# facebookresearch/SlowFast

Hardware: AMD Instinct MI355X
Metric: clips/sec (fwd+bwd), SlowFast-8x8-R50 32x224^2 synthetic clips, per-GPU batch 32 (higher is better)
Workload: dtype fp16; 1 GPU; SLOWFAST_8x8_R50: forward + cross_entropy loss + backward + sgd step, inputs resident in HBM, per-GPU batch 32; global_batch=32, parallelism=dp1, launch=hip-graph(fwd+bwd) + eager all-reduce/optimizer, optimizer=FlatOptimizer (fused unscale+norm+clip+update, dynamic loss scale on device)

## Files before the change

### include/sfamd.h

```cpp
#ifndef SFAMD_H
#define SFAMD_H
#include <stddef.h>
#include <stdint.h>
#ifdef __cplusplus
extern "C" {
#endif

#define SF_ABI_VERSION 35
typedef void* sf_stream_t;

typedef struct sf_conv_desc {
    int32_t N, Ci, Ti, Hi, Wi;
    int32_t Co, To, Ho, Wo;
    int32_t kT, kH, kW;
    int32_t sT, sH, sW;
    int32_t pT, pH, pW;
    int32_t dT, dH, dW;
    int32_t Cw;
    int32_t ldx, ldy;
    int32_t Cow;
} sf_conv_desc;

int sf_abi_version(void);
const char* sf_backend(void);
#define SF_ACT_FP16 0
#define SF_ACT_BF16_ID 1
int sf_act_dtype(void);
const char* sf_last_error(void);
const char* sf_build_id(void);

int sf_conv_weight_ld(const sf_conv_desc* d, int32_t* ldf, int32_t* ldd);
// ... 12 lines not shown
int sf_conv_fwd_mtiles(const sf_conv_desc* d);
int sf_conv_fwd(const sf_conv_desc* d, const void* x, const void* wf, const float* in_scale, const float* in_shift,
                int in_relu, const float* bias, void* y, float* stat_part, sf_stream_t stream);
int sf_conv_fwd_fused(const sf_conv_desc* d, const void* x, const void* wf, const float* bias, const void* resid,
                      int32_t ldr, int out_relu, void* y, sf_stream_t stream);
int sf_conv_dgrad(const sf_conv_desc* d, const void* dy, const void* wd, const void* resid, int32_t ldr,
                  const void* resid_bits, void* dx, sf_stream_t stream);
int sf_conv_dgrad_bn(const sf_conv_desc* d, const void* dy, const void* wd, const void* resid, int32_t ldr,
                     const void* resid_bits, void* dx, const float* mask_scale, const float* mask_shift,
                     const void* mask_bits, const void* bn_y, int32_t bn_ldy, float* bn_part, int32_t bn_part_rows,
                     int32_t* bn_rows, sf_stream_t stream);
int64_t sf_conv_wgrad_workspace(const sf_conv_desc* d);
int64_t sf_conv_wgrad_rowtab_bytes(const sf_conv_desc* d);
int sf_conv_wgrad_rowtab(const sf_conv_desc* d, void* tab, sf_stream_t stream);
int sf_conv_wgrad(const sf_conv_desc* d, const void* x, const float* in_scale, const float* in_shift, int in_relu,
                  const void* dy, float* dw, float out_scale, int zero_first, void* workspace, int64_t workspace_bytes,
                  const void* rowtab, sf_stream_t stream);
int sf_conv_c_bwd_plan(const sf_conv_desc* d, int in_affine, int mask_bits, int32_t* tile_rows, int64_t* workspace_bytes);
int sf_conv_c_bwd(const sf_conv_desc* d, const void* dz, int32_t lddz, const void* mask_bits, const void* yc, int32_t ldyc,
                  const float* coef, const void* act, const void* wd, const float* bn_scale, const float* bn_shift,
                  const void* bn_y, int32_t bn_ldy, float* bn_part, int32_t bn_part_rows, int32_t* bn_rows, void* d_in,
                  int32_t ld_in, float* dw, float out_scale, int zero_first, void* workspace, int64_t workspace_bytes,
                  sf_stream_t stream);

int sf_bn_finalize(float* part, int32_t nblk, int32_t C, int32_t Creal, float count, const float* gamma, const float* beta,
                   float* running_mean, float* running_var, float momentum, float eps, float* scale, float* shift,
                   float* save_mean, float* save_rstd, sf_stream_t stream);
int sf_bn_act(int64_t M, int32_t C, const void* y, int32_t ldy, const float* scale, const float* shift, const void* r,
              int32_t ldr, const float* rscale, const float* rshift, int relu, void* out, int32_t ldo, void* mask_out,
              sf_stream_t stream);
int sf_bn_bwd_blocks(int64_t M, int32_t C);
int sf_bn_bwd_reduce(int64_t M, int32_t C, const void* dz, int32_t lddz, const void* zmask, int32_t ldm, const void* y,
                     int32_t ldy, const float* scale, const float* shift, int relu_self, float* part,
                     sf_stream_t stream);
int sf_bn_bwd_finalize(float* part, int32_t nblk, int32_t C, int32_t Creal, float count, const float* gamma, const float* mean,
                       const float* rstd, float inv_loss_scale, float* dgamma, float* dbeta, int accumulate,
                       float* coef, sf_stream_t stream);
int sf_bn_bwd_apply(int64_t M, int32_t C, const void* dz, int32_t lddz, const void* zmask, int32_t ldm, const void* y,
                    int32_t ldy, const float* scale, const float* shift, int relu_self, const float* coef, void* dy,
                    int32_t lddy, void* gout, int32_t ldg, sf_stream_t stream);

int sf_pool_fwd(int32_t N, int32_t T, int32_t H, int32_t W, int32_t C, int32_t kH, int32_t kW, int32_t sH, int32_t sW,
                int32_t pH, int32_t pW, const void* y, int32_t ldy, const float* scale, const float* shift, int relu,
                void* out, int32_t ldo, void* argmax, int32_t cls, sf_stream_t stream);
int sf_pool_bwd(int32_t N, int32_t T, int32_t H, int32_t W, int32_t C, int32_t kH, int32_t kW, int32_t sH, int32_t sW,
                int32_t pH, int32_t pW, const void* pooled, int32_t ldp, const void* argmax, int relu,
// ... 262 lines not shown
```

### slowfast_amd/csrc/sf_api.hip

```cpp
#include "../../include/sfamd.h"
#include "sf_bn.h"
#include "sf_common.h"
#include "sf_igemm.h"
#include "sf_igemm2.h"
#include "sf_wgrad2.h"
#include "sf_cbwd.h"
#include "sf_pool.h"
#include "sf_dwconv.h"
#include "sf_dwsweep.h"
#include "sf_dwtemporal.h"
#include "sf_tokens.h"
#include "sf_x3d.h"
#include "sf_stem.h"
#include "sf_attn.h"
#include "sf_roi.h"
#include "sf_optim.h"
#include "sf_mixup.h"
#include "sf_erase.h"
#include "sf_pack.h"
#include "sf_sample.h"
#include "sf_color.h"
#include "sf_randaug.h"
#include "sf_sslcolor.h"
#include "sf_hog.h"
// ... 865 lines not shown
    int cip, cop, R;
    size_t ws_bytes;
};
#define SF_CBWD_MAX_WGS 1024
template <int CIP, int COP>
static void cbwd_fill(CbwdPlan& w) {
    using K = CbwdCfg<CIP, COP>;
    w.R = K::R;
    w.ws_bytes = (size_t)SF_CBWD_MAX_WGS * COP * CIP * 4;
}
#define SF_CBWD_FOR_SHAPE(cip, cop, ...)                                                         \
    do {                                                                                         \
        if ((cip) == 16 && (cop) == 32) { constexpr int CIP_ = 16, COP_ = 32; __VA_ARGS__; }            \
        else if ((cip) == 16 && (cop) == 64) { constexpr int CIP_ = 16, COP_ = 64; __VA_ARGS__; }       \
        else if ((cip) == 16 && (cop) == 128) { constexpr int CIP_ = 16, COP_ = 128; __VA_ARGS__; }     \
        else if ((cip) == 16 && (cop) == 256) { constexpr int CIP_ = 16, COP_ = 256; __VA_ARGS__; }     \
        else if ((cip) == 32 && (cop) == 32) { constexpr int CIP_ = 32, COP_ = 32; __VA_ARGS__; }       \
        else if ((cip) == 32 && (cop) == 64) { constexpr int CIP_ = 32, COP_ = 64; __VA_ARGS__; }       \
        else if ((cip) == 32 && (cop) == 128) { constexpr int CIP_ = 32, COP_ = 128; __VA_ARGS__; }     \
        else if ((cip) == 32 && (cop) == 256) { constexpr int CIP_ = 32, COP_ = 256; __VA_ARGS__; }     \
        else if ((cip) == 64 && (cop) == 32) { constexpr int CIP_ = 64, COP_ = 32; __VA_ARGS__; }       \
        else if ((cip) == 64 && (cop) == 64) { constexpr int CIP_ = 64, COP_ = 64; __VA_ARGS__; }       \
        else if ((cip) == 64 && (cop) == 128) { constexpr int CIP_ = 64, COP_ = 128; __VA_ARGS__; }     \
        else { constexpr int CIP_ = 64, COP_ = 256; __VA_ARGS__; }                                      \
    } while (0)
static CbwdPlan plan_cbwd(const sf_conv_desc* d, bool in_affine, bool mask_bits) {
    CbwdPlan w;
    memset(&w, 0, sizeof(w));
    if (test_hook("SF_CBWD", 1) == 0) return w;
    if (d->kT != 1 || d->kH != 1 || d->kW != 1 || d->sT != 1 || d->sH != 1 || d->sW != 1 || d->pT || d->pH || d->pW) return w;
    if (d->To != d->Ti || d->Ho != d->Hi || d->Wo != d->Wi) return w;
    if (d->Ci % 8 || d->Ci > 64 || d->Co % 32 || d->Co > 256) return w;
    if (in_affine || !mask_bits) return w;
    w.cip = d->Ci <= 16 ? 16 : d->Ci <= 32 ? 32 : 64;
    w.cop = d->Co <= 32 ? 32 : d->Co <= 64 ? 64 : d->Co <= 128 ? 128 : 256;
    SF_CBWD_FOR_SHAPE(w.cip, w.cop, (cbwd_fill<CIP_, COP_>(w)));
    w.ok = true;
    return w;
}

extern "C" int sf_conv_c_bwd_plan(const sf_conv_desc* d, int in_affine, int mask_bits, int32_t* tile_rows,
                                  int64_t* workspace_bytes) {
    if (check_desc(d)) return -1;
    const CbwdPlan w = plan_cbwd(d, in_affine != 0, mask_bits != 0);
    if (tile_rows) *tile_rows = w.ok ? 128 : 0;
    if (workspace_bytes) *workspace_bytes = w.ok ? (int64_t)w.ws_bytes : 0;
    return w.ok ? 1 : 0;
}
// ... 10 lines not shown
    REQUIRE(lddz >= d->Co && lddz % 8 == 0 && ldyc >= d->Co && ldyc % 8 == 0 && ld_in >= d->Ci && ld_in % 8 == 0,
            "sf_conv_c_bwd: bad row pitch");
    REQUIRE((((uintptr_t)dz | (uintptr_t)yc | (uintptr_t)act | (uintptr_t)wd | (uintptr_t)d_in | (uintptr_t)workspace) & 15) == 0,
            "sf_conv_c_bwd: operands must be 16-byte aligned");
    REQUIRE(workspace_bytes >= (int64_t)w.ws_bytes, "sf_conv_c_bwd: workspace too small (%lld < %lld bytes)",
            (long long)workspace_bytes, (long long)w.ws_bytes);
    const int64_t M = (int64_t)d->N * d->Ti * d->Hi * d->Wi;
    const int ntiles = cdiv(M, 128);
    const bool fuse = bn_part != nullptr;
    if (fuse) {
        REQUIRE(bn_scale && bn_shift && bn_y && bn_rows, "sf_conv_c_bwd: the fused reduction needs bn_scale, bn_shift, bn_y and bn_rows");
        REQUIRE(bn_ldy >= d->Ci && bn_ldy % 8 == 0 && ((uintptr_t)bn_y & 15) == 0, "sf_conv_c_bwd: bad bn_y pitch / alignment");
        REQUIRE(bn_part_rows >= ntiles, "sf_conv_c_bwd: the partial table needs ceil(positions / tile_rows) rows of [2][Ci] floats");
    }
    int32_t ldf, ldd;
    sf_conv_weight_ld(d, &ldf, &ldd);
    CbwdParams p;
    memset(&p, 0, sizeof(p));
    p.M = (int)M; p.Ci = d->Ci; p.Co = d->Co;
    p.dz = (const f16*)dz; p.lddz = lddz; p.bits = (const uint8_t*)mask_bits; p.yc = (const f16*)yc; p.ldyc = ldyc;
    p.coef = coef; p.act = (const f16*)act; p.ldact = d->ldx; p.wd = (const f16*)wd; p.ldw = ldd;
    if (fuse) { p.bnb_y = (const f16*)bn_y; p.bnb_ld = bn_ldy; p.bnb_scale = bn_scale; p.bnb_shift = bn_shift; p.bnb_part = bn_part; }
    p.dx = (f16*)d_in; p.lddx = ld_in; p.ws = (float*)workspace; p.tiles128 = ntiles;
    int wgs;
    const WgradPlan w2 = plan_conv_wgrad(d, false);
    const int forced = test_hook("SF_CBWD_WGS", 0);
    if (forced > 0) {
        wgs = forced < SF_CBWD_MAX_WGS ? forced : SF_CBWD_MAX_WGS;
        p.rps = roundup(cdiv(M, wgs), 32);
        wgs = cdiv(M, p.rps);
    } else if (w2.path == WGRAD_ROWTAB && w2.thin && w2.splits <= SF_CBWD_MAX_WGS) {
        wgs = w2.splits; p.rps = 0;
    } else {
        const WgradPlan w1 = plan_wgrad1(d);
        wgs = w1.splits; p.rps = w1.chunks_per_split * 32;
        REQUIRE(wgs <= SF_CBWD_MAX_WGS, "sf_conv_c_bwd: %d splits", wgs);
    }
    hipStream_t s = (hipStream_t)stream;
    SF_CBWD_FOR_SHAPE(w.cip, w.cop, hipLaunchKernelGGL((sf_cbwd_kernel<CIP_, COP_>), dim3(wgs), dim3(SF_THREADS), 0, s, p));
    if (check_launch("conv_c_bwd")) return -1;
    if (bn_rows) *bn_rows = fuse ? ntiles : 0;
    launch_wgrad_reduce(d, (const float*)workspace, wgs, w.cop, w.cip, false, dw, out_scale, zero_first, s);
    return check_launch("conv_c_bwd_reduce");
}

static RowTile make_rowtile(int64_t M, int C, int max_blocks, dim3& grid) {
    RowTile rt;
    rt.M = (int)M; rt.C = C;
    const int G = C / 8;
    const int TG = G < SF_THREADS ? G : SF_THREADS;
    const int rpi = SF_THREADS / TG;
    int passes = cdiv(M, (int64_t)rpi * max_blocks);
    if (passes < 1) passes = 1;
    rt.rows_per_block = rpi * passes;
    grid = dim3(cdiv(M, rt.rows_per_block), cdiv(G, SF_THREADS));
    return rt;
}
static int check_rows(const char* who, int64_t M, int C) {
    REQUIRE(M > 0 && M < (1ll << 31), "%s: bad row count", who);
    REQUIRE(C > 0 && C % 8 == 0, "%s: C must be a positive multiple of 8 (got %d)", who, C);
    return 0;
}

static const int kFoldAbove = tune_knob("SF_FOLD_ABOVE", 2048);
static int fold_partials(float* part, int& nblk, int C, hipStream_t s) {
    if (nblk <= kFoldAbove || nblk <= 256) return 1;
// ... 2470 lines not shown
```

### slowfast_amd/csrc/sf_cbwd.h

```cpp
#pragma once
#include "sf_bn.h"
#include "sf_common.h"
#include "sf_igemm.h"

struct CbwdParams {
    int M, Ci, Co;
    const f16* dz; int lddz;
    const uint8_t* bits;
    const f16* yc; int ldyc;
    const float* coef;
    const f16* act; int ldact;
    const f16* wd; int ldw;
    const f16* bnb_y; int bnb_ld;
    const float* bnb_scale; const float* bnb_shift;
    float* bnb_part;
    f16* dx; int lddx;
    float* ws;
    int rps;
    int tiles128;
};

template <int CIP, int COP>
struct CbwdCfg {
    static constexpr int R = COP >= 128 ? 64 : 128;
    static constexpr int NSUB = 128 / R;
    static constexpr int NJ = CIP / 16, KS = COP / 32, TI = R / 64;
    static constexpr int WAVES_M = COP == 32 ? 4 : 1, WAVES_C = 4 / WAVES_M;
    static constexpr int TC = COP / 16 / WAVES_C;
    static constexpr int KSM = R / WAVES_M / 32;
    static constexpr int LDY = COP + 8;
    static constexpr int CGO = COP / 8, RPP = SF_THREADS / CGO, NCH = R / RPP;
    static constexpr int ACH = CIP / 8, NACT = R * ACH / 64;
    static constexpr int NEPI = (R * ACH + SF_THREADS - 1) / SF_THREADS;
    static constexpr int DY_ELEMS = R * LDY, ACT_ELEMS = R * CIP, WD_ELEMS = CIP * LDY;
    static constexpr int RED_ELEMS = 4 * ACH * 24 * 2;
    static constexpr int UNION_ELEMS = DY_ELEMS > ACT_ELEMS + RED_ELEMS ? DY_ELEMS : ACT_ELEMS + RED_ELEMS;
    static constexpr int LDS_ELEMS = UNION_ELEMS + ACT_ELEMS + WD_ELEMS + 3 * COP * 2 + 2 * CIP * 2;
    static_assert(WAVES_M == 1 || LDS_ELEMS * 2 >= 4 * (COP / 16) * NJ * 256 * 4, "the cross-wave sum reuses the tile buffers");
    static constexpr int LDS_BYTES = LDS_ELEMS * 2;
    static constexpr int HELD = 4 * NJ * (TI + TC) + 9 * NCH + 4 * NEPI;
    static constexpr int OCC = HELD <= 72 ? 3 : 2;
    static_assert(R % 64 == 0 && R % RPP == 0 && NACT >= 1 && (R * ACH) % 64 == 0, "tile shape");
    static_assert(SF_THREADS % ACH == 0 && 64 % ACH == 0, "a thread keeps one d_in column group");
};

template <int CIP, int COP>
__global__ __launch_bounds__(SF_THREADS, (CbwdCfg<CIP, COP>::OCC)) void sf_cbwd_kernel(CbwdParams p) {
    using K = CbwdCfg<CIP, COP>;
    constexpr int R = K::R, LDY = K::LDY, NJ = K::NJ, TI = K::TI, TC = K::TC;
    __shared__ __attribute__((aligned(16))) f16 smem[K::LDS_ELEMS];
    f16* const DyL = smem;
    f16* const StL = smem;
    float* const red = reinterpret_cast<float*>(smem + K::ACT_ELEMS);
    f16* const ActL = smem + K::UNION_ELEMS;
    f16* const WdL = ActL + K::ACT_ELEMS;
    float* const coefL = reinterpret_cast<float*>(WdL + K::WD_ELEMS);
    float* const bnL = coefL + 3 * COP;

    const int tid = threadIdx.x;
    const int lane = tid & 63, wave = __builtin_amdgcn_readfirstlane(tid >> 6);
    const int pl = lane & 15, g4 = lane >> 4;
    const int G = (int)gridDim.x;
    const f16* const zline = reinterpret_cast<const f16*>(sf_zero_line);
    const bool bnb = p.bnb_part != nullptr;
// ... 9 lines not shown
        coefL[q] = c < p.Co ? p.coef[k * p.Co + c] : 0.f;
    }
    for (int q = tid; q < 2 * CIP; q += SF_THREADS) {
        const int k = q / CIP, c = q % CIP;
        bnL[q] = (bnb && c < p.Ci) ? (k ? p.bnb_shift[c] : p.bnb_scale[c]) : (k ? 0.f : 1.f);
    }

    const int scg = tid % K::CGO, srow = tid / K::CGO;
    const bool scol_ok = scg * 8 < p.Co;
    const int scgc = scol_ok ? scg : 0;
    const int ecg = tid % K::ACH;
    const bool ecol_ok = ecg * 8 < p.Ci;
    const int ecgc = ecol_ok ? ecg : 0;

    int r0 = 0, r1 = p.M, T0 = (int)blockIdx.x, Tstep = G, nwalk = 0;
    if (p.rps > 0) {
        r0 = (int)blockIdx.x * p.rps;
        r1 = r0 + p.rps < p.M ? r0 + p.rps : p.M;
        T0 = r0 >> 7;
        Tstep = 1;
        if (r1 > r0) nwalk = (((r1 + 127) >> 7) - T0) * K::NSUB;
    } else if (T0 < p.tiles128) nwalk = ((p.tiles128 - 1 - T0) / G + 1) * K::NSUB;
    auto tile_m0 = [&](int q) { return (T0 + (q / K::NSUB) * Tstep) * 128 + (q % K::NSUB) * R; };

    f16x8 dzr[K::NCH], ycr[K::NCH], ybr[K::NEPI];
    uint32_t mbr[K::NCH];
    auto load_regs = [&](int m0) {
#pragma unroll
        for (int u = 0; u < K::NCH; ++u) {
            int m = m0 + srow + u * K::RPP;
            if (m > p.M - 1) m = p.M - 1;
            dzr[u] = ld16(p.dz + (int64_t)m * p.lddz + scgc * 8);
            ycr[u] = ld16(p.yc + (int64_t)m * p.ldyc + scgc * 8);
            mbr[u] = p.bits[(int64_t)m * (p.Co >> 3) + scgc];
        }
    };
    auto load_yb = [&](int m0) {
#pragma unroll
        for (int e = 0; e < K::NEPI; ++e) {
            int m = m0 + (tid + e * SF_THREADS) / K::ACH;
            if (m > p.M - 1) m = p.M - 1;
            ybr[e] = ld16(p.bnb_y + (int64_t)m * p.bnb_ld + ecgc * 8);
        }
    };
    auto issue_act = [&](int m0) {
#pragma unroll
        for (int j = 0; j < (K::NACT + 3) / 4; ++j) {
            const int q = wave + 4 * j;
            if (q < K::NACT) {
                const int c = q * 64 + lane;
                const int m = m0 + c / K::ACH, cc = c % K::ACH;
                const f16* g = (m >= r0 && m < r1 && cc * 8 < p.Ci) ? p.act + (int64_t)m * p.ldact + cc * 8 : zline;
                SF_GLOBAL_LOAD_LDS16_ASM(g, ActL + q * 512);
            }
        }
    };


    f32x4 wacc[TC][NJ];
#pragma unroll
    for (int i = 0; i < TC; ++i)
#pragma unroll
        for (int j = 0; j < NJ; ++j) wacc[i][j] = (f32x4){0.f, 0.f, 0.f, 0.f};
    const int wc = wave % K::WAVES_C, wm = wave / K::WAVES_C;
    const int cobase = wc * TC * 16, mbase = wm * (R / K::WAVES_M);
    const int rowbase = wave * (R / 4);

    float bsg[8], bsgy[8];
#pragma unroll
    for (int e = 0; e < 8; ++e) { bsg[e] = 0.f; bsgy[e] = 0.f; }
    const int nq = nwalk;
    if (nq > 0) { load_regs(tile_m0(0)); issue_act(tile_m0(0)); }
    for (int q = 0; q < nq; ++q) {
        const int m0 = tile_m0(q);
        const int T = T0 + (q / K::NSUB) * Tstep;
// ... 64 lines not shown
            for (int i = 0; i < TI; ++i) {
                const f16x8 af = ld16(DyL + (rowbase + i * 16 + pl) * LDY + ks * 32 + 8 * g4);
#pragma unroll
                for (int j = 0; j < NJ; ++j) dacc[i][j] = SF_MFMA16(af, bf[j], dacc[i][j]);
            }
        }
        SF_BARRIER_KEEP_VMEM();
#pragma unroll
        for (int i = 0; i < TI; ++i)
#pragma unroll
            for (int j = 0; j < NJ; ++j)
#pragma unroll
                for (int r = 0; r < 4; ++r) StL[(rowbase + i * 16 + 4 * g4 + r) * CIP + j * 16 + pl] = (f16)dacc[i][j][r];
        SF_BARRIER_KEEP_VMEM();
        float bsc[8], bsh[8];
#pragma unroll
        for (int e = 0; e < 8; ++e) { bsc[e] = bnL[ecg * 8 + e]; bsh[e] = bnL[CIP + ecg * 8 + e]; }
#pragma unroll
        for (int e = 0; e < K::NEPI; ++e) {
            const int idx = tid + e * SF_THREADS;
            const int row = idx / K::ACH, m = m0 + row;
            if (idx < R * K::ACH && m < p.M && ecol_ok) {
                const f16x8 v = ld16(StL + row * CIP + ecg * 8);
                st16(p.dx + (int64_t)m * p.lddx + ecg * 8, v);
                if (bnb) bnb_accumulate(v, ybr[e], bsc, bsh, bsg, bsgy, false, 0u);
            }
        }
        if (bnb && q % K::NSUB == K::NSUB - 1) {
            bnb_reduce_store<4, K::ACH>(bsg, bsgy, red, p.bnb_part + (int64_t)T * 2 * p.Ci, 0, p.Ci);
#pragma unroll
            for (int e = 0; e < 8; ++e) { bsg[e] = 0.f; bsgy[e] = 0.f; }
        }
    }

    float* slab = p.ws + (int64_t)blockIdx.x * (COP * CIP);
    if constexpr (K::WAVES_M == 4) {
        __syncthreads();
        float* rd = reinterpret_cast<float*>(smem);
#pragma unroll
        for (int i = 0; i < TC; ++i)
#pragma unroll
            for (int j = 0; j < NJ; ++j)
#pragma unroll
                for (int r = 0; r < 4; ++r) rd[(((wave * TC + i) * NJ + j) * 4 + r) * 64 + lane] = wacc[i][j][r];
        __syncthreads();
        constexpr int TE = TC * NJ * 256;
        for (int e = tid; e < TE; e += SF_THREADS) {
// ... 15 lines not shown
```

### slowfast_amd/engine.py

```python
import functools
import os

import torch

from . import lib as _sflib

from . import ops

_f16 = _sflib.act_dtype()
_listeners = []
FORCE_WEIGHT_PREP = False
PARAM_EPOCH = 0
PACK_RECORD = None
PACK_PLAN = os.environ.get("SF_PACK_PLAN", "1") != "0"
BN_FUSE_REDUCE = os.environ.get("SF_BN_FUSE_REDUCE", "1") != "0"
CAT_IN_PLACE = os.environ.get("SF_CAT_IN_PLACE", "1") != "0"
SEGMENTS = None


class _Segments:
    def __init__(self):
        self.cuts = []

    def cut(self, tensors):
# ... 364 lines not shown
            dbeta, zb = _grad_dest(bn.bias)
            assert zg == zb
            return dgamma, dbeta, not zg
        return torch.empty_like(bn.weight), torch.empty_like(bn.bias), False

    def fused_c_geom(self, x):
        if self.bn is None or _sync_of(self.bn) is not None or not self.conv.weight.requires_grad:
            return None
        geom = self.geom(x.shape)
        return geom if ops.conv_c_bwd_plan(geom) is not None else None

    def fused_c_backward(self, geom, x, dz, y, st, bits, part=None, bn_fuse=None):
        bn = self.bn
        dgamma, dbeta, accumulate = self._bn_grad_dest()
        coef = ops.bn_bwd_coef(dz, y, bn.weight, st.mean, st.rstd, dgamma, dbeta, zmask=bits, inv_loss_scale=1.0,
                               accumulate=accumulate, part=part)
        dw, zero_first = _grad_dest(self.conv.weight)
        _, wd = self.weights(geom)
        fuse = None
        if bn_fuse is not None:
            y0, st0 = bn_fuse
            fuse = (y0, st0.scale, st0.shift)
        return ops.conv_c_bwd(dz, bits, y, coef, x, wd, geom, dw, bn=fuse, out_scale=1.0, zero_first=zero_first)

    def bn_backward(self, dz, y, st, zmask=None, relu_self=False, want_g=False, part=None):
        bn = self.bn
        dgamma, dbeta, accumulate = self._bn_grad_dest()
        return ops.bn_bwd(dz, y, bn.weight, st.mean, st.rstd, dgamma, dbeta, zmask=zmask,
                          relu_affine=(st.scale, st.shift) if relu_self else None, inv_loss_scale=1.0,
                          accumulate=accumulate, want_g=want_g, sync=_sync_of(bn), part=part)

    def params(self):
        p = [self.conv.weight]
        if self.conv.bias is not None:
            p.append(self.conv.bias)
        if self.bn is not None:
            p += [self.bn.weight, self.bn.bias]
        return p

    def _fold_source(self, w):
        return w

    def fold(self):
        w = self.conv.weight.detach().float()
        b = self.conv.bias.detach().float() if self.conv.bias is not None else None
        bn = self.bn
# ... 203 lines not shown
        ctx.mod = mod
        ctx.raw = (raw, y1, act, bits)
        ctx.bn = (bn, s1)
        ctx.save_for_backward(x)
        if BN_FUSE_REDUCE and tr:
            out._sf_block_bn = {"bits": bits, "y0": yc, "sync": _sync_of(units[-1].bn) is not None}
        return out

    @staticmethod
    @delivers_grads
    def backward(ctx, dout):
        mod = ctx.mod
        units, P = mod.branch2._chain, mod._proj
        (x,) = ctx.saved_tensors
        raw, y1, act, bits = ctx.raw
        bn, s1 = ctx.bn
        last = len(units) - 1
        part_c = tagged_bn_part(dout, raw[last])
        dout = as_cl(dout)
        need_dx = ctx.needs_input_grad[0]
        cgeom = units[last].fused_c_geom(act[last - 1]) if last > 0 else None
        if cgeom is None:
            dy = units[last].bn_backward(dout, raw[last], bn[last], zmask=bits, part=part_c)
        if P is not None:
            dy1 = P.bn_backward(dout, y1, s1, zmask=bits)
        for i in range(last, 0, -1):
            part = None
            if i == last and cgeom is not None:
                inner = (raw[i - 1], bn[i - 1]) if BN_FUSE_REDUCE and _sync_of(units[i - 1].bn) is None else None
                d_in, part = units[i].fused_c_backward(cgeom, act[i - 1], dout, raw[i], bn[i], bits, part=part_c, bn_fuse=inner)
            elif BN_FUSE_REDUCE and _sync_of(units[i - 1].bn) is None:
                d_in, part = units[i].backward(act[i - 1], None, dy, need_dx=True, bn_fuse=(raw[i - 1], bn[i - 1]))
            else:
                d_in = units[i].backward(act[i - 1], None, dy, need_dx=True)
            dy = units[i - 1].bn_backward(d_in, raw[i - 1], bn[i - 1], relu_self=True, part=part)
        prev = ctx.prev_bn if need_dx else None
        if prev is not None and prev["sync"]:
            prev = None
        if P is not None:
            dx1 = P.backward(x, None, dy1, need_dx=need_dx)
            dx = units[0].backward(x, None, dy, need_dx=need_dx, resid=dx1, bn_fuse=prev)
        else:
            dx = units[0].backward(x, None, dy, need_dx=need_dx, resid=dout, resid_bits=bits, bn_fuse=prev)
        if prev is not None:
            dx, pc = dx
            if pc is not None:
                tag_bn_part(dx, prev["y0"], pc)
        _notify(mod._param_list)
        ctx.raw = ctx.bn = ctx.prev_bn = None
        return (dx, None) + param_grads(ctx, 2)


CUT_BACKWARD = False
_cut_bn_tags = {}


def retag_cut_grad(g):
    tag = _cut_bn_tags.pop(g.data_ptr(), None)
    if tag is not None and getattr(g, "_sf_bn_part", None) is None and tag[2] == g.data_ptr() and tag[3] == g._version:
        g._sf_bn_part = tag


def tag_bn_part(dx, y0, part):
# ... 37 lines not shown
```

### slowfast_amd/lib.py

```python
import ctypes
import os
from ctypes import POINTER, Structure, c_char_p, c_float, c_int, c_int32, c_int64, c_void_p

_HERE = os.path.dirname(os.path.abspath(__file__))
ABI_VERSION = 35
ACT_MODE = os.environ.get("SF_ACT_DTYPE", "fp16").lower()
if ACT_MODE not in ("fp16", "bf16"):
    raise ValueError(f"SF_ACT_DTYPE={ACT_MODE!r}: expected fp16 or bf16")
DEFAULT_LIBRARY = os.path.join(_HERE, "libsfamd.so" if ACT_MODE == "fp16" else "libsfamd_bf16.so")


def act_dtype():
    import torch
    return torch.float16 if ACT_MODE == "fp16" else torch.bfloat16


def act_eps():
    return 2.0 ** -11 if ACT_MODE == "fp16" else 2.0 ** -8


class ConvDesc(Structure):

    _fields_ = [(n, c_int32) for n in (
        "N", "Ci", "Ti", "Hi", "Wi", "Co", "To", "Ho", "Wo", "kT", "kH", "kW", "sT", "sH", "sW",
        "pT", "pH", "pW", "dT", "dH", "dW", "Cw", "ldx", "ldy", "Cow")]


class PrepItem(Structure):
# ... 32 lines not shown
    "sf_abi_version": (c_int, []),
    "sf_backend": (c_char_p, []),
    "sf_act_dtype": (c_int, []),
    "sf_last_error": (c_char_p, []),
    "sf_build_id": (c_char_p, []),
    "sf_conv_weight_ld": (c_int, [POINTER(ConvDesc), POINTER(c_int32), POINTER(c_int32)]),
    "sf_prep_weights": (c_int, [POINTER(ConvDesc), _F, _P, _P, _P]),
    "sf_prep_item_fill": (c_int, [POINTER(ConvDesc), _F, _P, _P, POINTER(PrepItem)]),
    "sf_prep_item_blocks": (c_int64, [POINTER(PrepItem)]),
    "sf_prep_weights_batch": (c_int, [_P, _P, _P, c_int32, _P]),
    "sf_conv_fwd_mtiles": (c_int, [POINTER(ConvDesc)]),
    "sf_conv_fwd": (c_int, [POINTER(ConvDesc), _P, _P, _F, _F, c_int, _F, _P, _F, _P]),
    "sf_conv_fwd_fused": (c_int, [POINTER(ConvDesc), _P, _P, _F, _P, c_int32, c_int, _P, _P]),
    "sf_conv_dgrad": (c_int, [POINTER(ConvDesc), _P, _P, _P, c_int32, _P, _P, _P]),
    "sf_conv_dgrad_bn": (c_int, [POINTER(ConvDesc), _P, _P, _P, c_int32, _P, _P, _P, _P, _P, _P, c_int32, _P, c_int32,
                                 POINTER(c_int32), _P]),
    "sf_conv_wgrad_workspace": (c_int64, [POINTER(ConvDesc)]),
    "sf_conv_wgrad_rowtab_bytes": (c_int64, [POINTER(ConvDesc)]),
    "sf_conv_wgrad_rowtab": (c_int, [POINTER(ConvDesc), _P, _P]),
    "sf_conv_wgrad": (c_int, [POINTER(ConvDesc), _P, _F, _F, c_int, _P, _F, c_float, c_int, _P, c_int64, _P, _P]),
    "sf_conv_c_bwd_plan": (c_int, [POINTER(ConvDesc), c_int, c_int, POINTER(c_int32), POINTER(c_int64)]),
    "sf_conv_c_bwd": (c_int, [POINTER(ConvDesc), _P, c_int32, _P, _P, c_int32, _F, _P, _P, _F, _F, _P, c_int32, _F, c_int32,
                              POINTER(c_int32), _P, c_int32, _F, c_float, c_int, _P, c_int64, _P]),
    "sf_bn_finalize": (c_int, [_F, c_int32, c_int32, c_int32, c_float, _F, _F, _F, _F, c_float, c_float, _F, _F, _F, _F, _P]),
    "sf_bn_act": (c_int, [c_int64, c_int32, _P, c_int32, _F, _F, _P, c_int32, _F, _F, c_int, _P, c_int32, _P, _P]),
    "sf_bn_bwd_blocks": (c_int, [c_int64, c_int32]),
    "sf_flat_blocks": (c_int, [c_int64]),
    "sf_flat_sumsq": (c_int, [_F, c_int64, _F, _P]),
    "sf_step_control": (c_int, [_F, c_int32, _F, c_float, c_float, c_int, c_float, c_float, c_int32, _P]),
    "sf_flat_sgd": (c_int, [_F, _F, _F, _P, _P, _P, c_int32, _F, _P, _P, c_int32, c_float, c_float, c_float, c_int, _P]),
    "sf_flat_adamw": (c_int, [_F, _F, _F, _F, _P, _P, _P, c_int32, _F, _P, _P, c_int32, c_float, c_float, c_float, c_float, _P]),
    "sf_flat_sgd_tab": (c_int, [_F, _F, _F, _P, _P, _P, c_int32, _F, _F, _F, c_float, c_float, c_float, c_int, _P]),
    "sf_flat_adamw_tab": (c_int, [_F, _F, _F, _F, _P, _P, _P, c_int32, _F, _F, _F, c_float, c_float, c_float, c_float, _P]),
    "sf_flat_lars_trust": (c_int, [_F, _F, _P, _P, _P, c_int32, _P, c_int32, _F, _F, _P, _F, c_float, c_float, c_float, _P]),
    "sf_bn_bwd_reduce": (c_int, [c_int64, c_int32, _P, c_int32, _P, c_int32, _P, c_int32, _F, _F, c_int, _F, _P]),
    "sf_bn_bwd_finalize": (c_int, [_F, c_int32, c_int32, c_int32, c_float, _F, _F, _F, c_float, _F, _F, c_int, _F, _P]),
    "sf_bn_bwd_apply": (c_int, [c_int64, c_int32, _P, c_int32, _P, c_int32, _P, c_int32, _F, _F, c_int, _F, _P,
                                c_int32, _P, c_int32, _P]),
    "sf_pool_fwd": (c_int, [c_int32] * 11 + [_P, c_int32, _F, _F, c_int, _P, c_int32, _P, c_int32, _P]),
    "sf_pool_bwd": (c_int, [c_int32] * 11 + [_P, c_int32, _P, c_int, _P, c_int32, _P, c_int32, c_int32, _P]),
    "sf_pool3d_fwd": (c_int, [c_int32] * 8 + [_P, c_int32, _P, c_int32, _P, _P]),
    "sf_pool3d_bwd": (c_int, [c_int32] * 8 + [_P, _P, c_int32, _P, c_int32, _P]),
    "sf_ncthw_to_cl": (c_int, [_F, c_int32, c_int32, c_int64, c_int32, _P, _P]),
    "sf_cl_to_ncthw": (c_int, [_P, c_int32, c_int32, c_int32, c_int64, _F, _P]),
    "sf_bgemm": (c_int, [c_int64, c_int32, c_int32, _P, c_int32, _P, c_int32, _F, _P, c_int32, _P, c_int32, c_int32,
                         c_int32] + [c_int64] * 8 + [c_int32, c_float, _P]),
# ... 182 lines not shown
```

### slowfast_amd/ops.py

```python
from ctypes import byref, c_int32, c_int64

import torch

from . import lib as _sflib

from .lib import ConvDesc, SfError, get_lib

_f16 = _sflib.act_dtype()


def _triple(v):
    return tuple(v) if isinstance(v, (tuple, list)) else (v, v, v)


def _stream(t):
    if t.is_cuda:
        return torch.cuda.current_stream(t.device).cuda_stream
    if get_lib().backend != "hostsim":
        raise SfError("slowfast_amd kernels need CUDA/HIP tensors (got a CPU tensor and the gfx950 library)")
    return None


def _ptr(t):
    return None if t is None else t.data_ptr()
# ... 372 lines not shown
    M = rows(yc)
    assert bits.dtype == torch.uint8 and bits.is_contiguous() and bits.numel() == M * (geom.Co // 8)
    assert coef.dtype == torch.float32 and coef.is_contiguous() and tuple(coef.shape) == (3, geom.Co)
    d_in = cl_empty(geom.in_shape, dz.device) if out is None else out
    assert tuple(d_in.shape) == geom.in_shape
    part, cap, nrows = None, 0, c_int32(0)
    y0 = sc = sh = None
    if bn is not None:
        y0, sc, sh = bn
        assert tuple(y0.shape) == geom.in_shape
        cap = (M + tile_rows - 1) // tile_rows
        part = torch.empty((cap, 2, geom.Ci), dtype=torch.float32, device=dz.device)
    ws = _workspace(dz.device, ws_bytes)
    W = 2.0 * M * geom.Co
    get_lib().call("sf_conv_c_bwd", byref(geom.desc(cl_ld(act), geom.Co)), dz.data_ptr(), cl_ld(dz), bits.data_ptr(), yc.data_ptr(),
                   cl_ld(yc), coef.data_ptr(), act.data_ptr(), wd.data_ptr(), _ptr(sc), _ptr(sh), _ptr(y0),
                   cl_ld(y0) if y0 is not None else 0, _ptr(part), cap, byref(nrows), d_in.data_ptr(), cl_ld(d_in), dw.data_ptr(),
                   float(out_scale), int(zero_first), ws.data_ptr(), ws.numel(), _stream(dz),
                   work=dict(flops=4.0 * M * geom.Co * geom.Cw,
                             bytes=W * (2 + 1 / 16) + 2.0 * M * geom.Ci * (2 + int(bn is not None))))
    return d_in, (part[:nrows.value] if part is not None and nrows.value > 0 else None)


def _pool_args(y, kernel, stride, padding):
    N, C, T, H, W = y.shape
    (kH, kW), (sH, sW), (pH, pW) = kernel, stride, padding
    return (N, T, H, W, C, kH, kW, sH, sW, pH, pW), ((H + 2 * pH - kH) // sH + 1, (W + 2 * pW - kW) // sW + 1)


def pool_fwd(y, kernel, stride, padding, affine=None, want_argmax=True):
    args, (Ho, Wo) = _pool_args(y, kernel, stride, padding)
    N, C, T, H, W = y.shape
    out = cl_empty((N, C, T, Ho, Wo), y.device)
    arg = torch.empty((N, T, Ho, Wo, C), dtype=torch.uint8, device=y.device) if want_argmax else None
    sc, sh, relu = _affine(affine)
    get_lib().call("sf_pool_fwd", *args, y.data_ptr(), cl_ld(y), _ptr(sc), _ptr(sh), relu, out.data_ptr(),
                   cl_ld(out), _ptr(arg), 0, _stream(y), work=dict(bytes=2.0 * (y.numel() + out.numel())))
    return out, arg


def pool_bwd(in_shape, pooled, argmax, dout, kernel, stride, padding, relu=True):
    N, C, T, H, W = in_shape
    (kH, kW), (sH, sW), (pH, pW) = kernel, stride, padding
    assert tuple(dout.shape) == tuple(pooled.shape)
    g = cl_empty(in_shape, dout.device)
    get_lib().call("sf_pool_bwd", N, T, H, W, C, kH, kW, sH, sW, pH, pW, pooled.data_ptr(), cl_ld(pooled),
# ... 4 lines not shown
```

Measured before the change: 907.9 clips/s.

## Fuse projection shortcut BN backward, wgrad and dgrad into one cbwd kernel

Adds sf_conv_proj_bwd, which reuses the fused conv_c backward kernel for the residual projection shortcut (1x1 conv, stride 1 or 2 spatially, Ci up to 128). The kernel applies BN backward, computes dgrad and wgrad partials, and for stride 2 scatters dx into every other row while writing zeros to the skipped positions. This replaces the separate bn_bwd_apply, wgrad and dgrad launches and removes the round trip of the intermediate dy1 through memory. The catch is the new CIP=128 instantiations, which may have lower occupancy because of LDS, and scattered 16-byte stores on the stride-2 path.

```diff
diff --git a/include/sfamd.h b/include/sfamd.h
--- a/include/sfamd.h
+++ b/include/sfamd.h
@@ -6,7 +6,7 @@
 extern "C" {
 #endif
 
-#define SF_ABI_VERSION 35
+#define SF_ABI_VERSION 36
 typedef void* sf_stream_t;
 
 typedef struct sf_conv_desc {
@@ -65,6 +65,10 @@
                   const void* bn_y, int32_t bn_ldy, float* bn_part, int32_t bn_part_rows, int32_t* bn_rows, void* d_in,
                   int32_t ld_in, float* dw, float out_scale, int zero_first, void* workspace, int64_t workspace_bytes,
                   sf_stream_t stream);
+int sf_conv_proj_bwd_plan(const sf_conv_desc* d, int in_affine, int mask_bits, int64_t* workspace_bytes);
+int sf_conv_proj_bwd(const sf_conv_desc* d, const void* dz, int32_t lddz, const void* mask_bits, const void* y1, int32_t ldy1,
+                     const float* coef, const void* x, const void* wd, void* d_in, int32_t ld_in, float* dw, float out_scale,
+                     int zero_first, void* workspace, int64_t workspace_bytes, sf_stream_t stream);
 
 int sf_bn_finalize(float* part, int32_t nblk, int32_t C, int32_t Creal, float count, const float* gamma, const float* beta,
                    float* running_mean, float* running_var, float momentum, float eps, float* scale, float* shift,
diff --git a/slowfast_amd/csrc/sf_api.hip b/slowfast_amd/csrc/sf_api.hip
--- a/slowfast_amd/csrc/sf_api.hip
+++ b/slowfast_amd/csrc/sf_api.hip
@@ -911,8 +911,28 @@
         else if ((cip) == 64 && (cop) == 32) { constexpr int CIP_ = 64, COP_ = 32; __VA_ARGS__; }       \
         else if ((cip) == 64 && (cop) == 64) { constexpr int CIP_ = 64, COP_ = 64; __VA_ARGS__; }       \
         else if ((cip) == 64 && (cop) == 128) { constexpr int CIP_ = 64, COP_ = 128; __VA_ARGS__; }     \
-        else { constexpr int CIP_ = 64, COP_ = 256; __VA_ARGS__; }                                      \
+        else if ((cip) == 64 && (cop) == 256) { constexpr int CIP_ = 64, COP_ = 256; __VA_ARGS__; }     \
+        else if ((cip) == 128 && (cop) == 32) { constexpr int CIP_ = 128, COP_ = 32; __VA_ARGS__; }     \
+        else if ((cip) == 128 && (cop) == 64) { constexpr int CIP_ = 128, COP_ = 64; __VA_ARGS__; }     \
+        else if ((cip) == 128 && (cop) == 128) { constexpr int CIP_ = 128, COP_ = 128; __VA_ARGS__; }   \
+        else { constexpr int CIP_ = 128, COP_ = 256; __VA_ARGS__; }                                     \
     } while (0)
+static int cbwd_deal_rows(const sf_conv_desc* d, int64_t M, int* rps) {
+    const WgradPlan w2 = plan_conv_wgrad(d, false);
+    const int forced = test_hook("SF_CBWD_WGS", 0);
+    if (forced > 0) {
+        const int wgs = forced < SF_CBWD_MAX_WGS ? forced : SF_CBWD_MAX_WGS;
+        *rps = roundup(cdiv(M, wgs), 32);
+        return cdiv(M, *rps);
+    }
+    if (w2.path == WGRAD_ROWTAB && w2.thin && w2.splits <= SF_CBWD_MAX_WGS) {
+        *rps = 0;
+        return w2.splits;
+    }
+    const WgradPlan w1 = plan_wgrad1(d);
+    *rps = w1.chunks_per_split * 32;
+    return w1.splits;
+}
 static CbwdPlan plan_cbwd(const sf_conv_desc* d, bool in_affine, bool mask_bits) {
     CbwdPlan w;
     memset(&w, 0, sizeof(w));
@@ -969,26 +989,74 @@
     p.coef = coef; p.act = (const f16*)act; p.ldact = d->ldx; p.wd = (const f16*)wd; p.ldw = ldd;
     if (fuse) { p.bnb_y = (const f16*)bn_y; p.bnb_ld = bn_ldy; p.bnb_scale = bn_scale; p.bnb_shift = bn_shift; p.bnb_part = bn_part; }
     p.dx = (f16*)d_in; p.lddx = ld_in; p.ws = (float*)workspace; p.tiles128 = ntiles;
-    int wgs;
-    const WgradPlan w2 = plan_conv_wgrad(d, false);
-    const int forced = test_hook("SF_CBWD_WGS", 0);
-    if (forced > 0) {
-        wgs = forced < SF_CBWD_MAX_WGS ? forced : SF_CBWD_MAX_WGS;
-        p.rps = roundup(cdiv(M, wgs), 32);
-        wgs = cdiv(M, p.rps);
-    } else if (w2.path == WGRAD_ROWTAB && w2.thin && w2.splits <= SF_CBWD_MAX_WGS) {
-        wgs = w2.splits; p.rps = 0;
-    } else {
-        const WgradPlan w1 = plan_wgrad1(d);
-        wgs = w1.splits; p.rps = w1.chunks_per_split * 32;
-        REQUIRE(wgs <= SF_CBWD_MAX_WGS, "sf_conv_c_bwd: %d splits", wgs);
-    }
+    const int wgs = cbwd_deal_rows(d, M, &p.rps);
+    REQUIRE(wgs <= SF_CBWD_MAX_WGS, "sf_conv_c_bwd: %d splits", wgs);
     hipStream_t s = (hipStream_t)stream;
     SF_CBWD_FOR_SHAPE(w.cip, w.cop, hipLaunchKernelGGL((sf_cbwd_kernel<CIP_, COP_>), dim3(wgs), dim3(SF_THREADS), 0, s, p));
     if (check_launch("conv_c_bwd")) return -1;
     if (bn_rows) *bn_rows = fuse ? ntiles : 0;
     launch_wgrad_reduce(d, (const float*)workspace, wgs, w.cop, w.cip, false, dw, out_scale, zero_first, s);
     return check_launch("conv_c_bwd_reduce");
+}
+
+static CbwdPlan plan_proj_bwd(const sf_conv_desc* d, bool in_affine, bool mask_bits) {
+    CbwdPlan w;
+    memset(&w, 0, sizeof(w));
+    if (test_hook("SF_CBWD", 1) == 0) return w;
+    if (d->kT != 1 || d->kH != 1 || d->kW != 1 || d->pT || d->pH || d->pW || d->dT != 1 || d->dH != 1 || d->dW != 1) return w;
+    const bool unit = d->sH == 1 && d->sW == 1 && d->Ho == d->Hi && d->Wo == d->Wi;
+    const bool half = d->sH == 2 && d->sW == 2 && d->Hi == 2 * d->Ho && d->Wi == 2 * d->Wo;
+    if (d->sT != 1 || d->To != d->Ti || !(unit || half)) return w;
+    if (d->Ci % 8 || d->Ci > 128 || d->Co % 32 || d->Co > 256) return w;
+    if (in_affine || !mask_bits) return w;
+    w.cip = d->Ci <= 16 ? 16 : d->Ci <= 32 ? 32 : d->Ci <= 64 ? 64 : 128;
+    w.cop = d->Co <= 32 ? 32 : d->Co <= 64 ? 64 : d->Co <= 128 ? 128 : 256;
+    int rps;
+    const int wgs = cbwd_deal_rows(d, (int64_t)d->N * d->To * d->Ho * d->Wo, &rps);
+    if (wgs > SF_CBWD_MAX_WGS) return w;
+    w.R = 128;
+    w.ws_bytes = (size_t)wgs * w.cop * w.cip * 4;
+    w.ok = true;
+    return w;
+}
+
+extern "C" int sf_conv_proj_bwd_plan(const sf_conv_desc* d, int in_affine, int mask_bits, int64_t* workspace_bytes) {
+    if (check_desc(d)) return -1;
+    const CbwdPlan w = plan_proj_bwd(d, in_affine != 0, mask_bits != 0);
+    if (workspace_bytes) *workspace_bytes = w.ok ? (int64_t)w.ws_bytes : 0;
+    return w.ok ? 1 : 0;
+}
+
+extern "C" int sf_conv_proj_bwd(const sf_conv_desc* d, const void* dz, int32_t lddz, const void* mask_bits, const void* y1,
+                                int32_t ldy1, const float* coef, const void* x, const void* wd, void* d_in, int32_t ld_in,
+                                float* dw, float out_scale, int zero_first, void* workspace, int64_t workspace_bytes,
+                                sf_stream_t stream) {
+    if (check_desc(d)) return -1;
+    REQUIRE(dz && mask_bits && y1 && coef && x && wd && d_in && dw && workspace, "sf_conv_proj_bwd: null pointer");
+    const CbwdPlan w = plan_proj_bwd(d, false, true);
+    REQUIRE(w.ok, "sf_conv_proj_bwd: this geometry keeps sf_bn_bwd_apply + sf_conv_wgrad + sf_conv_dgrad (sf_conv_proj_bwd_plan == 0)");
+    REQUIRE(lddz >= d->Co && lddz % 8 == 0 && ldy1 >= d->Co && ldy1 % 8 == 0 && ld_in >= d->Ci && ld_in % 8 == 0 &&
+            d->ldx >= d->Ci && d->ldx % 8 == 0, "sf_conv_proj_bwd: bad row pitch");
+    REQUIRE((((uintptr_t)dz | (uintptr_t)y1 | (uintptr_t)x | (uintptr_t)wd | (uintptr_t)d_in | (uintptr_t)workspace) & 15) == 0,
+            "sf_conv_proj_bwd: operands must be 16-byte aligned");
+    REQUIRE(workspace_bytes >= (int64_t)w.ws_bytes, "sf_conv_proj_bwd: workspace too small (%lld < %lld bytes)",
+            (long long)workspace_bytes, (long long)w.ws_bytes);
+    const int64_t M = (int64_t)d->N * d->To * d->Ho * d->Wo;
+    int32_t ldf, ldd;
+    sf_conv_weight_ld(d, &ldf, &ldd);
+    CbwdParams p;
+    memset(&p, 0, sizeof(p));
+    p.M = (int)M; p.Ci = d->Ci; p.Co = d->Co;
+    p.dz = (const f16*)dz; p.lddz = lddz; p.bits = (const uint8_t*)mask_bits; p.yc = (const f16*)y1; p.ldyc = ldy1;
+    p.coef = coef; p.act = (const f16*)x; p.ldact = d->ldx; p.wd = (const f16*)wd; p.ldw = ldd;
+    p.dx = (f16*)d_in; p.lddx = ld_in; p.ws = (float*)workspace; p.tiles128 = cdiv(M, 128);
+    p.str2 = d->sH == 2 ? 1 : 0; p.fdWo = make_fastdiv(d->Wo);
+    const int wgs = cbwd_deal_rows(d, M, &p.rps);
+    hipStream_t s = (hipStream_t)stream;
+    SF_CBWD_FOR_SHAPE(w.cip, w.cop, hipLaunchKernelGGL((sf_cbwd_kernel<CIP_, COP_>), dim3(wgs), dim3(SF_THREADS), 0, s, p));
+    if (check_launch("conv_proj_bwd")) return -1;
+    launch_wgrad_reduce(d, (const float*)workspace, wgs, w.cop, w.cip, false, dw, out_scale, zero_first, s);
+    return check_launch("conv_proj_bwd_reduce");
 }
 
 static RowTile make_rowtile(int64_t M, int C, int max_blocks, dim3& grid) {
diff --git a/slowfast_amd/csrc/sf_cbwd.h b/slowfast_amd/csrc/sf_cbwd.h
--- a/slowfast_amd/csrc/sf_cbwd.h
+++ b/slowfast_amd/csrc/sf_cbwd.h
@@ -18,6 +18,8 @@
     float* ws;
     int rps;
     int tiles128;
+    int str2;
+    FastDiv fdWo;
 };
 
 template <int CIP, int COP>
@@ -39,7 +41,9 @@
     static_assert(WAVES_M == 1 || LDS_ELEMS * 2 >= 4 * (COP / 16) * NJ * 256 * 4, "the cross-wave sum reuses the tile buffers");
     static constexpr int LDS_BYTES = LDS_ELEMS * 2;
     static constexpr int HELD = 4 * NJ * (TI + TC) + 9 * NCH + 4 * NEPI;
-    static constexpr int OCC = HELD <= 72 ? 3 : 2;
+    static constexpr int OCC_REGS = HELD <= 72 ? 3 : 2;
+    static constexpr int OCC_LDS = 160 * 1024 / LDS_BYTES;
+    static constexpr int OCC = OCC_LDS < OCC_REGS ? OCC_LDS : OCC_REGS;
     static_assert(R % 64 == 0 && R % RPP == 0 && NACT >= 1 && (R * ACH) % 64 == 0, "tile shape");
     static_assert(SF_THREADS % ACH == 0 && 64 % ACH == 0, "a thread keeps one d_in column group");
 };
@@ -95,6 +99,13 @@
         if (r1 > r0) nwalk = (((r1 + 127) >> 7) - T0) * K::NSUB;
     } else if (T0 < p.tiles128) nwalk = ((p.tiles128 - 1 - T0) / G + 1) * K::NSUB;
     auto tile_m0 = [&](int q) { return (T0 + (q / K::NSUB) * Tstep) * 128 + (q % K::NSUB) * R; };
+    const int Wi = 2 * (int)p.fdWo.d;
+    auto in_row = [&](int m) -> int64_t {
+        if (!p.str2) return m;
+        uint32_t qr, wo;
+        fd_divmod((uint32_t)m, p.fdWo, qr, wo);
+        return (int64_t)qr * (2 * Wi) + 2 * wo;
+    };
 
     f16x8 dzr[K::NCH], ycr[K::NCH], ybr[K::NEPI];
     uint32_t mbr[K::NCH];
@@ -123,7 +134,7 @@
             if (q < K::NACT) {
                 const int c = q * 64 + lane;
                 const int m = m0 + c / K::ACH, cc = c % K::ACH;
-                const f16* g = (m >= r0 && m < r1 && cc * 8 < p.Ci) ? p.act + (int64_t)m * p.ldact + cc * 8 : zline;
+                const f16* g = (m >= r0 && m < r1 && cc * 8 < p.Ci) ? p.act + in_row(m) * p.ldact + cc * 8 : zline;
                 SF_GLOBAL_LOAD_LDS16_ASM(g, ActL + q * 512);
             }
         }
@@ -234,7 +245,13 @@
             const int row = idx / K::ACH, m = m0 + row;
             if (idx < R * K::ACH && m < p.M && ecol_ok) {
                 const f16x8 v = ld16(StL + row * CIP + ecg * 8);
-                st16(p.dx + (int64_t)m * p.lddx + ecg * 8, v);
+                f16* const o = p.dx + in_row(m) * p.lddx + ecg * 8;
+                st16(o, v);
+                if (p.str2) {
+                    st16(o + p.lddx, zero8());
+                    st16(o + (int64_t)Wi * p.lddx, zero8());
+                    st16(o + (int64_t)(Wi + 1) * p.lddx, zero8());
+                }
                 if (bnb) bnb_accumulate(v, ybr[e], bsc, bsh, bsg, bsgy, false, 0u);
             }
         }
diff --git a/slowfast_amd/engine.py b/slowfast_amd/engine.py
--- a/slowfast_amd/engine.py
+++ b/slowfast_amd/engine.py
@@ -410,6 +410,21 @@
             y0, st0 = bn_fuse
             fuse = (y0, st0.scale, st0.shift)
         return ops.conv_c_bwd(dz, bits, y, coef, x, wd, geom, dw, bn=fuse, out_scale=1.0, zero_first=zero_first)
+
+    def fused_proj_geom(self, x):
+        if self.bn is None or _sync_of(self.bn) is not None or not self.conv.weight.requires_grad:
+            return None
+        geom = self.geom(x.shape)
+        return geom if ops.conv_proj_bwd_plan(geom) is not None else None
+
+    def fused_proj_backward(self, geom, x, dz, y, st, bits):
+        bn = self.bn
+        dgamma, dbeta, accumulate = self._bn_grad_dest()
+        coef = ops.bn_bwd_coef(dz, y, bn.weight, st.mean, st.rstd, dgamma, dbeta, zmask=bits, inv_loss_scale=1.0,
+                               accumulate=accumulate)
+        dw, zero_first = _grad_dest(self.conv.weight)
+        _, wd = self.weights(geom)
+        return ops.conv_proj_bwd(dz, bits, y, coef, x, wd, geom, dw, out_scale=1.0, zero_first=zero_first)
 
     def bn_backward(self, dz, y, st, zmask=None, relu_self=False, want_g=False, part=None):
         bn = self.bn
@@ -659,7 +674,10 @@
         cgeom = units[last].fused_c_geom(act[last - 1]) if last > 0 else None
         if cgeom is None:
             dy = units[last].bn_backward(dout, raw[last], bn[last], zmask=bits, part=part_c)
-        if P is not None:
+        pgeom = P.fused_proj_geom(x) if P is not None and need_dx else None
+        if pgeom is not None:
+            dx1 = P.fused_proj_backward(pgeom, x, dout, y1, s1, bits)
+        elif P is not None:
             dy1 = P.bn_backward(dout, y1, s1, zmask=bits)
         for i in range(last, 0, -1):
             part = None
@@ -675,7 +693,8 @@
         if prev is not None and prev["sync"]:
             prev = None
         if P is not None:
-            dx1 = P.backward(x, None, dy1, need_dx=need_dx)
+            if pgeom is None:
+                dx1 = P.backward(x, None, dy1, need_dx=need_dx)
             dx = units[0].backward(x, None, dy, need_dx=need_dx, resid=dx1, bn_fuse=prev)
         else:
             dx = units[0].backward(x, None, dy, need_dx=need_dx, resid=dout, resid_bits=bits, bn_fuse=prev)
diff --git a/slowfast_amd/lib.py b/slowfast_amd/lib.py
--- a/slowfast_amd/lib.py
+++ b/slowfast_amd/lib.py
@@ -3,7 +3,7 @@
 from ctypes import POINTER, Structure, c_char_p, c_float, c_int, c_int32, c_int64, c_void_p
 
 _HERE = os.path.dirname(os.path.abspath(__file__))
-ABI_VERSION = 35
+ABI_VERSION = 36
 ACT_MODE = os.environ.get("SF_ACT_DTYPE", "fp16").lower()
 if ACT_MODE not in ("fp16", "bf16"):
     raise ValueError(f"SF_ACT_DTYPE={ACT_MODE!r}: expected fp16 or bf16")
@@ -82,6 +82,9 @@
     "sf_conv_c_bwd_plan": (c_int, [POINTER(ConvDesc), c_int, c_int, POINTER(c_int32), POINTER(c_int64)]),
     "sf_conv_c_bwd": (c_int, [POINTER(ConvDesc), _P, c_int32, _P, _P, c_int32, _F, _P, _P, _F, _F, _P, c_int32, _F, c_int32,
                               POINTER(c_int32), _P, c_int32, _F, c_float, c_int, _P, c_int64, _P]),
+    "sf_conv_proj_bwd_plan": (c_int, [POINTER(ConvDesc), c_int, c_int, POINTER(c_int64)]),
+    "sf_conv_proj_bwd": (c_int, [POINTER(ConvDesc), _P, c_int32, _P, _P, c_int32, _F, _P, _P, _P, c_int32, _F, c_float, c_int, _P,
+                                 c_int64, _P]),
     "sf_bn_finalize": (c_int, [_F, c_int32, c_int32, c_int32, c_float, _F, _F, _F, _F, c_float, c_float, _F, _F, _F, _F, _P]),
     "sf_bn_act": (c_int, [c_int64, c_int32, _P, c_int32, _F, _F, _P, c_int32, _F, _F, c_int, _P, c_int32, _P, _P]),
     "sf_bn_bwd_blocks": (c_int, [c_int64, c_int32]),
diff --git a/slowfast_amd/ops.py b/slowfast_amd/ops.py
--- a/slowfast_amd/ops.py
+++ b/slowfast_amd/ops.py
@@ -418,6 +418,32 @@
     return d_in, (part[:nrows.value] if part is not None and nrows.value > 0 else None)
 
 
+def conv_proj_bwd_plan(geom, in_affine=False, mask_bits=True):
+    ws = c_int64(0)
+    ok = get_lib().call("sf_conv_proj_bwd_plan", byref(geom.desc(geom.Ci, geom.Co)), int(bool(in_affine)), int(bool(mask_bits)),
+                        byref(ws))
+    return ws.value if ok == 1 else None
+
+
+def conv_proj_bwd(dz, bits, y1, coef, x, wd, geom, dw, out_scale=1.0, zero_first=True, out=None):
+    ws_bytes = conv_proj_bwd_plan(geom)
+    assert ws_bytes is not None, "conv_proj_bwd: the planner rejects this geometry"
+    assert tuple(x.shape) == geom.in_shape and tuple(dz.shape) == geom.out_shape and tuple(y1.shape) == geom.out_shape
+    assert dw.dtype == torch.float32 and dw.is_contiguous() and dw.numel() == geom.Cow * geom.Cw * geom.taps
+    M = rows(y1)
+    assert bits.dtype == torch.uint8 and bits.is_contiguous() and bits.numel() == M * (geom.Co // 8)
+    assert coef.dtype == torch.float32 and coef.is_contiguous() and tuple(coef.shape) == (3, geom.Co)
+    d_in = cl_empty(geom.in_shape, dz.device) if out is None else out
+    assert tuple(d_in.shape) == geom.in_shape
+    ws = _workspace(dz.device, ws_bytes)
+    get_lib().call("sf_conv_proj_bwd", byref(geom.desc(cl_ld(x), geom.Co)), dz.data_ptr(), cl_ld(dz), bits.data_ptr(), y1.data_ptr(),
+                   cl_ld(y1), coef.data_ptr(), x.data_ptr(), wd.data_ptr(), d_in.data_ptr(), cl_ld(d_in), dw.data_ptr(),
+                   float(out_scale), int(zero_first), ws.data_ptr(), ws.numel(), _stream(dz),
+                   work=dict(flops=4.0 * M * geom.Co * geom.Cw,
+                             bytes=2.0 * M * geom.Co * (2 + 1 / 16) + 2.0 * M * geom.Ci + 2.0 * rows(d_in) * geom.Ci))
+    return d_in
+
+
 def _pool_args(y, kernel, stride, padding):
     N, C, T, H, W = y.shape
     (kH, kW), (sH, sW), (pH, pW) = kernel, stride, padding
```

New measurement: 918.9 clips/s, median of 6. 1.01x the previous value.
